# BVE-Reborn/rend3

Hardware: AMD Instinct MI355X
Metric: shaded Mpixels/s @4K (whole frame: cull+compact all cameras, 4 shadow views, PBR opaque, tonemap) (higher is better)
Workload: dtype f32; 1 GPU; BASELINE.json configs[2] stand-in: bistro_like (seed 0xB157, every object owns its geometry), 3840x2160, full PBR opaque + 4 directional shadow views (2048^2), camera dolly, 130 materials with base colour + normal + AO/roughness/metallic maps (RGBA8, mips, trilinear); objects=3000, triangles=2823212, cameras=5, parallelism=single GPU

## Files before the change

### bindings/rend3-amd-sys/src/lib.rs

```rust
#![allow(non_camel_case_types, non_upper_case_globals, clippy::too_many_arguments)]
use std::os::raw::{c_char, c_int, c_void};

pub const R3N_OK: i32 = 0;
pub const R3N_ERR_INVALID_ARG: i32 = -1;
pub const R3N_ERR_HIP: i32 = -2;
pub const R3N_ERR_NO_DEVICE: i32 = -3;
pub const R3N_ERR_STATE: i32 = -4;
pub const R3N_ERR_UNSUPPORTED: i32 = -5;
pub const R3N_ERR_CAPACITY: i32 = -6;
pub const R3N_CAMERA_VIEWPORT: u32 = 0xFFFFFFFF;
pub const R3N_MAX_SHADOW_VIEWS: u32 = 64;
pub const R3N_PASS_DEPTH: u32 = 0;
pub const R3N_PASS_FORWARD: u32 = 1;
pub const R3N_SOURCE_PREDICTED: u32 = 0;
pub const R3N_SOURCE_RESIDUAL: u32 = 1;
pub const R3N_KEY_OPAQUE: u32 = 0;
pub const R3N_KEY_CUTOUT: u32 = 1;
pub const R3N_KEY_BLEND: u32 = 2;
pub const R3N_TEXTURE_RGBA8_UNORM: u32 = 0;
pub const R3N_TEXTURE_RGBA8_UNORM_SRGB: u32 = 1;
pub const R3N_TEXTURE_R8_UNORM: u32 = 2;
pub const R3N_TEXTURE_RG8_UNORM: u32 = 3;
pub const R3N_TEXTURE_BGRA8_UNORM: u32 = 4;
pub const R3N_TEXTURE_BGRA8_UNORM_SRGB: u32 = 5;
// ... 427 lines not shown
    pub fn r3n_output_buffer(ctx: *mut r3n_ctx, rgba8: *mut *mut c_void, bytes: *mut u64) -> c_int;
    pub fn r3n_output_buffer_async(ctx: *mut r3n_ctx, rgba8: *mut *mut c_void, bytes: *mut u64, stream: *mut *mut c_void) -> c_int;
    pub fn r3n_output_work_enqueued(ctx: *mut r3n_ctx) -> c_int;
    pub fn r3n_readback_visible_objects(ctx: *mut r3n_ctx, camera: u32, flags: *mut u8, capacity: u32) -> c_int;
    pub fn r3n_readback_triangle_sets(ctx: *mut r3n_ctx, camera: u32, pass: *mut u8, residual: *mut u8, n: u64) -> c_int;
    pub fn r3n_readback_draw_calls(ctx: *mut r3n_ctx, camera: u32, calls: *mut r3n_indirect_call) -> c_int;
    pub fn r3n_readback_raster_stats(ctx: *mut r3n_ctx, big_items: *mut u32) -> c_int;
    pub fn r3n_readback_blend_order(ctx: *mut r3n_ctx, order: *mut u32, rank_base: *mut u32, capacity: u32) -> c_int;
    pub fn r3n_readback_baked(ctx: *mut r3n_ctx, camera: u32, model_view_and_mvp: *mut f32, capacity: u32) -> c_int;
    pub fn r3n_readback_mesh(ctx: *mut r3n_ctx, byte_offset: u64, dst: *mut c_void, bytes: u64) -> c_int;
    pub fn r3n_readback_joint_matrices(ctx: *mut r3n_ctx, first_matrix: u32, dst: *mut f32, n_matrices: u32) -> c_int;
    pub fn r3n_readback_texture_descs(ctx: *mut r3n_ctx, descs: *mut r3n_texture_desc32, capacity: u32, n_slots: *mut u32) -> c_int;
    pub fn r3n_readback_texels(ctx: *mut r3n_ctx, first_texel: u64, rgba8: *mut u32, n_texels: u64) -> c_int;
    pub fn r3n_readback_visibility(ctx: *mut r3n_ctx, keys: *mut u64) -> c_int;
    pub fn r3n_readback_depth(ctx: *mut r3n_ctx, depth: *mut f32) -> c_int;
    pub fn r3n_readback_hiz(ctx: *mut r3n_ctx, pyramid: *mut f32, count: u64) -> c_int;
    pub fn r3n_readback_shadow_atlas(ctx: *mut r3n_ctx, atlas: *mut f32) -> c_int;
    pub fn r3n_readback_hdr(ctx: *mut r3n_ctx, rgba16f: *mut u16) -> c_int;
    pub fn r3n_readback_output(ctx: *mut r3n_ctx, rgba8: *mut u8, rgba_f32: *mut f32) -> c_int;
    pub fn r3n_timing_enable(ctx: *mut r3n_ctx, enable: c_int) -> c_int;
    pub fn r3n_timing_overhead(ctx: *mut r3n_ctx, ms_per_span: *mut f64) -> c_int;
    pub fn r3n_set_multi_stream(ctx: *mut r3n_ctx, enable: c_int) -> c_int;
    pub fn r3n_stage_times(ctx: *mut r3n_ctx, ms: *mut f64, launches: *mut u64, reset: c_int) -> c_int;
    pub fn r3n_hbm_copy_rate(ctx: *mut r3n_ctx, bytes: u64, repeats: u32, gb_per_s: *mut f64) -> c_int;
    pub fn r3n_selftest_exact_math(hip_device: c_int, hist: *mut u64, guarded: *mut u64) -> c_int;
    pub fn r3n_selftest_unorm8(hip_device: c_int, n_bad: *mut u32) -> c_int;
    pub fn r3n_host_mat4_mul(a: *const f32, b: *const f32, out: *mut f32);
    pub fn r3n_host_mat4_inverse(m: *const f32, out: *mut f32);
    pub fn r3n_host_look_at(eye: *const f32, center: *const f32, up: *const f32, rh: c_int, out: *mut f32);
    pub fn r3n_host_projection(kind: c_int, params: *const f32, rh: c_int, aspect_ratio: f32, out: *mut f32);
    pub fn r3n_host_frustum_from_matrix(m: *const f32, planes20: *mut f32);
    pub fn r3n_host_frustum_contains_sphere(planes20: *const f32, center: *const f32, radius: f32) -> c_int;
    pub fn r3n_host_bounding_sphere_from_mesh(positions: *const f32, vertex_count: u64, out_center: *mut f32, out_radius: *mut f32);
    pub fn r3n_host_bounding_sphere_apply_transform(center: *const f32, radius: f32, m: *const f32, out_center: *mut f32, out_radius: *mut f32);
    pub fn r3n_host_build_object_records(n: u32, transforms: *const f32, mesh_desc: *const f32, mesh_u32: *const u32, material_index: *const u32, out_records: *mut r3n_object128);
    pub fn r3n_host_calculate_normals(positions: *const f32, vertex_count: u64, indices: *const u32, index_count: u64, left_handed: c_int, normals: *mut f32);
    pub fn r3n_host_calculate_tangents(positions: *const f32, normals: *const f32, uvs: *const f32, vertex_count: u64, indices: *const u32, index_count: u64, tangents: *mut f32);
    pub fn r3n_host_vertex_adjacency(indices: *const u32, index_count: u64, vertex_count: u64, out: *mut u32) -> c_int;
    pub fn r3n_host_shadow_camera(direction: *const f32, distance: f32, resolution: u32, camera_location: *const f32, rh: c_int, out_view: *mut f32, out_proj: *mut f32);
    pub fn r3n_host_allocate_shadow_atlas(handles: *const u32, resolutions: *const u16, n: u32, max_dimension: u32, out_dimensions: *mut u32, out_maps: *mut u32) -> u32;
    pub fn r3n_host_evaluate_frame(camera: *const r3n_host_camera144, lights: *const r3n_host_directional_light48, n_lights: u32, max_atlas_dimension: u32, ambient: *const f32, width: u32, height: u32, samples: u32, object_capacity: u32, out: *mut r3n_host_frame) -> c_int;
}
```

### include/r3n.h

```cpp
#ifndef R3N_H
#define R3N_H

#include <stdint.h>

#ifdef __cplusplus
extern "C" {
#endif

#define R3N_OK 0
#define R3N_ERR_INVALID_ARG (-1)
#define R3N_ERR_HIP (-2)
#define R3N_ERR_NO_DEVICE (-3)
#define R3N_ERR_STATE (-4)
#define R3N_ERR_UNSUPPORTED (-5)
#define R3N_ERR_CAPACITY (-6)

typedef uint32_t r3n_camera;
#define R3N_CAMERA_VIEWPORT 0xFFFFFFFFu
#define R3N_MAX_SHADOW_VIEWS 64u

#define R3N_PASS_DEPTH 0u
#define R3N_PASS_FORWARD 1u
#define R3N_SOURCE_PREDICTED 0u
#define R3N_SOURCE_RESIDUAL 1u
// ... 325 lines not shown
#define R3N_STAGE_CLEAR 7
#define R3N_STAGE_RASTER_BIG 8
#define R3N_STAGE_SHADOW_RASTER 9
#define R3N_STAGE_SHADOW_RASTER_BIG 10
#define R3N_STAGE_SKINNING 11
#define R3N_STAGE_VERTEX 12
#define R3N_STAGE_POSE 13
#define R3N_STAGE_EXCHANGE_SHADOW 14
#define R3N_STAGE_EXCHANGE_DEPTH 15
#define R3N_STAGE_EXCHANGE_ROWS 16
#define R3N_STAGE_EXCHANGE_KEYS 17
#define R3N_STAGE_RASTER_CUT 18
#define R3N_STAGE_RASTER_BIG_CUT 19
#define R3N_STAGE_SKYBOX 20
#define R3N_STAGE_BLEND_SORT 21
#define R3N_STAGE_MORPH 22
#define R3N_STAGE_NORMALS 23
#define R3N_STAGE_TANGENTS 24
#define R3N_STAGE_COUNT 25
int r3n_timing_enable(r3n_ctx *ctx, int enable);
int r3n_timing_overhead(r3n_ctx *ctx, double *ms_per_span);
int r3n_set_multi_stream(r3n_ctx *ctx, int enable);
int r3n_stage_times(r3n_ctx *ctx, double ms[R3N_STAGE_COUNT], uint64_t launches[R3N_STAGE_COUNT], int reset);
int r3n_hbm_copy_rate(r3n_ctx *ctx, uint64_t bytes, uint32_t repeats, double *gb_per_s);
int r3n_selftest_exact_math(int hip_device, unsigned long long *hist, unsigned long long *guarded);
int r3n_selftest_unorm8(int hip_device, uint32_t *n_bad);

void r3n_host_mat4_mul(const float *a, const float *b, float *out);
void r3n_host_mat4_inverse(const float *m, float *out);
void r3n_host_look_at(const float eye[3], const float center[3], const float up[3], int rh, float *out);
void r3n_host_projection(int kind, const float *params, int rh, float aspect_ratio, float *out);
void r3n_host_frustum_from_matrix(const float *m, float *planes20);
int r3n_host_frustum_contains_sphere(const float *planes20, const float center[3], float radius);
void r3n_host_bounding_sphere_from_mesh(const float *positions, uint64_t vertex_count, float out_center[3],
                                        float *out_radius);
void r3n_host_bounding_sphere_apply_transform(const float center[3], float radius, const float *m,
                                              float out_center[3], float *out_radius);
void r3n_host_build_object_records(uint32_t n, const float *transforms , const float *mesh_desc ,
                                   const uint32_t *mesh_u32 , const uint32_t *material_index ,
                                   r3n_object128 *out_records);
void r3n_host_calculate_normals(const float *positions, uint64_t vertex_count, const uint32_t *indices,
                                uint64_t index_count, int left_handed, float *normals);
void r3n_host_calculate_tangents(const float *positions, const float *normals, const float *uvs, uint64_t vertex_count,
                                 const uint32_t *indices, uint64_t index_count, float *tangents);
int r3n_host_vertex_adjacency(const uint32_t *indices, uint64_t index_count, uint64_t vertex_count, uint32_t *out);
void r3n_host_shadow_camera(const float direction[3], float distance, uint32_t resolution,
// ... 42 lines not shown
```

### rend3_amd/_ffi.py

```python
import ctypes
import os

import numpy as np

from . import build as _build

vp = ctypes.c_void_p
u32 = ctypes.c_uint32
u64 = ctypes.c_uint64
cint = ctypes.c_int
cfloat = ctypes.c_float

CAMERA_VIEWPORT = 0xFFFFFFFF
PASS_DEPTH, PASS_FORWARD = 0, 1
SOURCE_PREDICTED, SOURCE_RESIDUAL = 0, 1
KEY_OPAQUE, KEY_CUTOUT, KEY_BLEND = 0, 1, 2
STAGES = ["bake", "object_cull", "triangle_cull", "hiz", "raster", "shade", "tonemap", "clear", "raster_big",
          "shadow_raster", "shadow_raster_big", "skinning", "vertex", "pose", "exchange_shadow", "exchange_depth", "exchange_rows", "exchange_keys",
          "raster_cut", "raster_big_cut", "skybox", "blend_sort"]
STAGE_NAMES = STAGES + ["morph", "normals"]
STAGE_TABLE = STAGE_NAMES + ["tangents"]

COMM_ID_BYTES, COMM_IDS = 128, 3

# ... 53 lines not shown
    "r3n_exchange_depth": (cint, [vp, vp, vp]),
    "r3n_set_row_range": (cint, [vp, u32, u32]),
    "r3n_output_buffer": (cint, [vp, vp, vp]),
    "r3n_output_buffer_async": (cint, [vp, vp, vp, vp]),
    "r3n_output_work_enqueued": (cint, [vp]),
    "r3n_readback_visible_objects": (cint, [vp, u32, vp, u32]),
    "r3n_readback_triangle_sets": (cint, [vp, u32, vp, vp, u64]),
    "r3n_readback_draw_calls": (cint, [vp, u32, vp]),
    "r3n_readback_raster_stats": (cint, [vp, vp]),
    "r3n_readback_blend_order": (cint, [vp, vp, vp, u32]),
    "r3n_readback_baked": (cint, [vp, u32, vp, u32]),
    "r3n_readback_mesh": (cint, [vp, u64, vp, u64]),
    "r3n_readback_texture_descs": (cint, [vp, vp, u32, vp]),
    "r3n_readback_texels": (cint, [vp, u64, vp, u64]),
    "r3n_readback_joint_matrices": (cint, [vp, u32, vp, u32]),
    "r3n_readback_visibility": (cint, [vp, vp]),
    "r3n_readback_depth": (cint, [vp, vp]),
    "r3n_readback_hiz": (cint, [vp, vp, u64]),
    "r3n_readback_shadow_atlas": (cint, [vp, vp]),
    "r3n_readback_hdr": (cint, [vp, vp]),
    "r3n_readback_output": (cint, [vp, vp, vp]),
    "r3n_timing_enable": (cint, [vp, cint]),
    "r3n_stage_times": (cint, [vp, vp, vp, cint]),
    "r3n_set_multi_stream": (cint, [vp, cint]),
    "r3n_hbm_copy_rate": (cint, [vp, u64, u32, vp]),
    "r3n_selftest_exact_math": (cint, [cint, vp, vp]),
    "r3n_selftest_unorm8": (cint, [cint, vp]),
    "r3n_host_mat4_mul": (None, [vp, vp, vp]),
    "r3n_host_mat4_inverse": (None, [vp, vp]),
    "r3n_host_look_at": (None, [vp, vp, vp, cint, vp]),
    "r3n_host_projection": (None, [cint, vp, cint, cfloat, vp]),
    "r3n_host_frustum_from_matrix": (None, [vp, vp]),
    "r3n_host_frustum_contains_sphere": (cint, [vp, vp, cfloat]),
    "r3n_host_bounding_sphere_from_mesh": (None, [vp, u64, vp, vp]),
    "r3n_host_bounding_sphere_apply_transform": (None, [vp, cfloat, vp, vp, vp]),
    "r3n_host_build_object_records": (None, [u32, vp, vp, vp, vp, vp]),
    "r3n_host_calculate_normals": (None, [vp, u64, vp, u64, cint, vp]),
    "r3n_host_calculate_tangents": (None, [vp, vp, vp, u64, vp, u64, vp]),
    "r3n_host_vertex_adjacency": (cint, [vp, u64, u64, vp]),
    "r3n_host_shadow_camera": (None, [vp, cfloat, u32, vp, cint, vp, vp]),
    "r3n_host_allocate_shadow_atlas": (u32, [vp, vp, u32, u32, vp, vp]),
    "r3n_host_evaluate_frame": (cint, [vp, vp, u32, u32, vp, u32, u32, u32, u32, vp]),
}

MAX_SHADOW_VIEWS = 64
MAX_MORPH_TARGETS = 256
# ... 90 lines not shown
```

### rend3_amd/csrc/kernels_shade.h

```cpp
#pragma once
#include <type_traits>

#include "device_math.h"
#include "texture.h"

#define R3N_TEX_OCC 5
#define R3N_MS_OCC 4

struct TriRecord;
struct ViewLights;
struct ShadeArgs {
    const unsigned long long *vis;
    uint32_t width, height, row_begin, row_end;
    const r3n_frame_uniforms496 *fu;
    const r3n_camera_header240 *hdr;
    const r3n_object128 *objects;
    const uint32_t *mesh;
    const r3n_baked128 *baked;
    const r3n_material208 *materials;
    uint32_t n_materials;
    const uint32_t *tri_base;
    const uint32_t *slot_table;
    uint32_t slot_table_size;
    const uint8_t *dir_buf;
    const uint8_t *point_buf;
    const float *atlas;
    uint32_t atlas_w, atlas_h;
    float clear[4];
    ushort4 *hdr_out;
    uchar4 *ldr_out;
    const unsigned char *srgb_lut;
    bool out_bgr;
    TextureArgs tex;
    ushort4 *samples_out;
    TriRecord *tri_rec;
    unsigned char *seen;
    uint32_t total_tris;
    uint32_t *edge_list, *edge_count;
    uint32_t edge_capacity;
    const ViewLights *view_lights;
    const uint32_t *material_feat;
    uint32_t variants;
    uint32_t resolve_lds;
};
#define R3N_EDGEQ 32u

#define R3N_FEAT_TEX_ALBEDO   0x001u
#define R3N_FEAT_TEX_NORMAL   0x002u
#define R3N_FEAT_TEX_AOMR     0x004u
#define R3N_FEAT_TEX_AOMR_X   0x008u
#define R3N_FEAT_TEX_MISC     0x010u
#define R3N_FEAT_VCOLOR       0x020u
#define R3N_FEAT_UNLIT        0x040u
#define R3N_FEAT_NEAREST      0x080u
#define R3N_FEAT_AOMR_SPLIT   0x100u
#define R3N_FEAT_CLEARCOAT    0x200u
#define R3N_FEAT_NORMAL_FLAGS 0x400u
#define R3N_FEAT_ALBEDO_OFF   0x800u
#define R3N_FEAT_TEX_GENERAL  0x1000u
#define R3N_FEAT_ALL          0x1FFFu
#define R3N_BATCH_OCC 4
#define R3N_CLS_PLAIN  0u
#define R3N_CLS_ALBEDO (R3N_FEAT_TEX_ALBEDO)
#define R3N_CLS_PBR3   (R3N_FEAT_TEX_ALBEDO | R3N_FEAT_TEX_NORMAL | R3N_FEAT_TEX_AOMR)
#define R3N_CLS_ALL    R3N_FEAT_ALL
#define R3N_VARIANTS 4u
static inline uint32_t r3n_material_features(const r3n_material208 &m) {
    const uint32_t f = m.flags;
// ... 228 lines not shown
R3N_DEV uchar4 tonemap_half4(const unsigned char *__restrict__ lut, ushort4 h, bool bgr = false) {
    const float al = (float)__builtin_bit_cast(_Float16, h.w);
    const float a = (!(al > 0.0f)) ? 0.0f : (al >= 1.0f ? 1.0f : al);
    const unsigned char r = srgb8_of_half(lut, h.x), g = srgb8_of_half(lut, h.y), b = srgb8_of_half(lut, h.z);
    return make_uchar4(bgr ? b : r, g, bgr ? r : b, (unsigned char)(a * 255.0f + 0.5f));
}
R3N_DEV float srgb_scene_to_display(float x) {
    const float e = x > 0.0031308f ? 1.055f * powf(x, 0.4166f) - 0.055f : x * 12.92f;
    if (!(e > 0.0f)) return 0.0f;
    return e >= 1.0f ? 1.0f : e;
}

R3N_DEV ushort4 pack_half4(const float v[4]) {
    ushort4 o;
    o.x = __builtin_bit_cast(unsigned short, (_Float16)v[0]);
    o.y = __builtin_bit_cast(unsigned short, (_Float16)v[1]);
    o.z = __builtin_bit_cast(unsigned short, (_Float16)v[2]);
    o.w = __builtin_bit_cast(unsigned short, (_Float16)v[3]);
    return o;
}


template <bool TEX>
R3N_DEV void vertex_stage(const ShadeArgs &a, uint32_t id, TriRecord &r) {
    const uint32_t slot = id - 1u;
    const uint32_t bucket = slot >> R3N_SLOT_TABLE_SHIFT;
    uint32_t lo = a.slot_table[bucket];
    uint32_t hi = bucket + 1u < a.slot_table_size ? a.slot_table[bucket + 1u] + 1u : a.hdr->object_count;
    while (hi - lo > 1u) {
        const uint32_t mid = lo + (hi - lo) / 2u;
        if (a.tri_base[mid] <= slot) lo = mid; else hi = mid;
    }
    const uint32_t obj = lo, tri = slot - a.tri_base[obj];
    const r3n_object128 &ob = a.objects[obj];
    const uint4 of0 = *reinterpret_cast<const uint4 *>(reinterpret_cast<const char *>(&ob) + 80);
    const uint4 of1 = *reinterpret_cast<const uint4 *>(reinterpret_cast<const char *>(&ob) + 96);
    const uint32_t of5 = ob.vertex_attribute_start_offsets[5];
    const uint32_t mat_index = of0.z < a.n_materials ? of0.z : 0u;
    const r3n_material208 &mat = a.materials[mat_index];
    const float *mv = a.baked[obj].model_view;
    r.object = obj;
    r.material = mat_index;
    r.feat = a.material_feat != nullptr ? a.material_feat[mat_index] : R3N_FEAT_ALL;

    uint32_t idx[3];
    float p[3][4];
    const float inv_s2[3] = {1.0f / dot3(mv, mv), 1.0f / dot3(mv + 4, mv + 4), 1.0f / dot3(mv + 8, mv + 8)};
    const uint32_t first = of0.x + tri * 3u;
    const uint32_t pos_off = of0.w;
    const uint32_t nrm_off = of1.x;
    const uint32_t tan_off = of1.y;
    const uint32_t uv0_off = of1.z;
    const uint32_t col_off = of5;
    bool any_tex = false, normal_map = false;
    if (TEX) {
        const uint4 t0 = *reinterpret_cast<const uint4 *>(&mat.textures[0]), t1 = *reinterpret_cast<const uint4 *>(&mat.textures[4]);
// ... 22 lines not shown
        } else {
            r.vt[k][0] = r.vt[k][1] = r.vt[k][2] = 0.0f;
        }
        if (col_off != R3N_INVALID) {
            const uint32_t cw = a.mesh[col_off / 4u + idx[k]];
#pragma unroll
            for (int c = 0; c < 4; ++c) r.vc[k][c] = (float)((cw >> (8 * c)) & 0xFFu) / 255.0f;
        } else {
#pragma unroll
            for (int c = 0; c < 4; ++c) r.vc[k][c] = 1.0f;
        }
        if (TEX && any_tex) fetch_uv0(a.mesh, uv0_off, idx[k], r.uv[k]);
        else r.uv[k][0] = r.uv[k][1] = 0.0f;
    }
    TriSetup ts;
    setup_triangle(p, (float)a.width / 2.0f, (float)a.height / 2.0f,
                   (a.hdr->flags & R3N_PCU_POSITIVE_AREA_VISIBLE) != 0u, ts);
#pragma unroll
    for (int i = 0; i < 3; ++i)
#pragma unroll
        for (int c = 0; c < 3; ++c) r.e[i][c] = ts.e[i][c];
}

template <class M> R3N_DEV f2 interp2(const float lam[3], f2 a0, f2 a1, f2 a2) {
    return M::mad(splat2(lam[2]), a2, M::mad(splat2(lam[1]), a1, splat2(lam[0]) * a0));
}
template <class M> R3N_DEV float interp1(const float lam[3], float a0, float a1, float a2) {
    return M::mad(lam[2], a2, M::mad(lam[1], a1, lam[0] * a0));
}
template <class M> R3N_DEV void interp_vec3(const float lam[3], const float a[3][3], float o[3]) {
    const f2 xy = interp2<M>(lam, (f2){a[0][0], a[0][1]}, (f2){a[1][0], a[1][1]}, (f2){a[2][0], a[2][1]});
    o[0] = xy.x; o[1] = xy.y;
    o[2] = interp1<M>(lam, a[0][2], a[1][2], a[2][2]);
}
template <class M> R3N_DEV void interp_vec4(const float lam[3], const float a[3][4], float o[4]) {
    const f2 xy = interp2<M>(lam, (f2){a[0][0], a[0][1]}, (f2){a[1][0], a[1][1]}, (f2){a[2][0], a[2][1]});
    const f2 zw = interp2<M>(lam, (f2){a[0][2], a[0][3]}, (f2){a[1][2], a[1][3]}, (f2){a[2][2], a[2][3]});
    o[0] = xy.x; o[1] = xy.y; o[2] = zw.x; o[3] = zw.y;
}

template <class T, bool SL> R3N_DEV T load_light(const T *p) {
#if defined(__HIP_DEVICE_COMPILE__)
    if (SL) {
        static_assert(sizeof(T) % 4 == 0, "whole dwords");
        const unsigned long long v = (unsigned long long)p;
        const uint32_t lo = (uint32_t)__builtin_amdgcn_readfirstlane((uint32_t)v), hi = (uint32_t)__builtin_amdgcn_readfirstlane((uint32_t)(v >> 32));
// ... 258 lines not shown
R3N_DEV void shade_fragment(const ShadeArgs &a, const LdsDirLight *s_dir, const LdsPointLight *s_point, uint32_t n_dir,
                            uint32_t n_point, uint32_t id, uint32_t x, uint32_t y, float out[4]) {
    TriRecord r;
    vertex_stage<TEX>(a, id, r);
    fragment_stage<TEX, M>(a, s_dir, s_point, n_dir, n_point, r, x, y, out);
}

static __global__ __launch_bounds__(256) void k_mark_visible(const unsigned long long *__restrict__ vis, unsigned char *__restrict__ seen,
                                                      size_t first_pixel, size_t n_pixels) {
    const size_t i = (size_t)blockIdx.x * 256u + threadIdx.x;
    const uint32_t id = i < n_pixels ? (uint32_t)(vis[first_pixel + i] & 0xFFFFFFFFull) : 0u;
    const uint32_t left = (uint32_t)__builtin_amdgcn_update_dpp((int)~id, (int)id, 0x111, 0xF, 0xF, false);
    if (id != 0u && id != left) seen[id - 1u] = 1;
}
template <bool TEX>
__global__ __launch_bounds__(256) void k_vertex_stage(ShadeArgs a) {
    const uint32_t slot = blockIdx.x * 256u + threadIdx.x;
    if (slot >= a.total_tris || !a.seen[slot]) return;
    a.seen[slot] = 0;
    TriRecord r;
    vertex_stage<TEX>(a, slot + 1u, r);
    r._pad[0] = r._pad[1] = r._pad[2] = r._pad[3] = 0u;
    a.tri_rec[slot] = r;
}

R3N_DEV void stage_lights(const ShadeArgs &a, LdsDirLight *s_dir, LdsPointLight *s_point, uint32_t &n_dir, uint32_t &n_point) {
    n_dir = min(*reinterpret_cast<const uint32_t *>(a.dir_buf), (uint32_t)R3N_MAX_DIR_LIGHTS);
    n_point = min(*reinterpret_cast<const uint32_t *>(a.point_buf), (uint32_t)R3N_MAX_POINT_LIGHTS);

    const r3n_dir_light128 *dirs = reinterpret_cast<const r3n_dir_light128 *>(a.dir_buf + 16);
    const r3n_point_light32 *points = reinterpret_cast<const r3n_point_light32 *>(a.point_buf + 16);
    for (uint32_t i = threadIdx.x; i < n_dir * 4u; i += 256u) {
        const uint32_t li = i >> 2, c = i & 3u;
        const float *col = a.fu->inv_view + 4 * c;
        float o[4];
        mul_vec4(dirs[li].view_proj, col[0], col[1], col[2], col[3], o);
#pragma unroll
        for (int r = 0; r < 4; ++r) s_dir[li].m[4 * c + r] = o[r];
        if (c == 0) {
            const float nd[3] = {-dirs[li].direction[0], -dirs[li].direction[1], -dirs[li].direction[2]};
            float l[3];
            mat3_mul_vec3(a.fu->view, a.fu->view + 4, a.fu->view + 8, nd, l);
            normalize3(l);
#pragma unroll
            for (int r = 0; r < 3; ++r) { s_dir[li].l[r] = l[r]; s_dir[li].color[r] = dirs[li].color[r]; }
            s_dir[li].sane = (fabsf(dirs[li].color[0]) <= 1e6f && fabsf(dirs[li].color[1]) <= 1e6f && fabsf(dirs[li].color[2]) <= 1e6f &&
// ... 349 lines not shown
    } else {
        h[0] = hdr[i0];
        h[1] = two ? hdr[i0 + 1u] : make_ushort4(0, 0, 0, 0);
    }
    uchar4 o8[2];
#pragma unroll
    for (int k = 0; k < 2; ++k) {
        o8[k] = tonemap_half4(srgb_lut, h[k], bgr);
        if (out_f32 != nullptr && (k == 0 || two)) {
            const float r = (float)__builtin_bit_cast(_Float16, h[k].x), g = (float)__builtin_bit_cast(_Float16, h[k].y);
            const float b = (float)__builtin_bit_cast(_Float16, h[k].z), al = (float)__builtin_bit_cast(_Float16, h[k].w);
            out_f32[i0 + (size_t)k] = make_float4(manual ? srgb_scene_to_display(r) : srgb_oetf(r), manual ? srgb_scene_to_display(g) : srgb_oetf(g),
                                                  manual ? srgb_scene_to_display(b) : srgb_oetf(b),
                                                  (!(al > 0.0f)) ? 0.0f : (al >= 1.0f ? 1.0f : al));
        }
    }
    out[i0] = o8[0];
    if (two) out[i0 + 1u] = o8[1];
}
#endif

extern "C" {
int r3n_internal_build_srgb_lut(unsigned char *lut, hipStream_t stream);
int r3n_internal_shade_prepass(const ShadeArgs *a, int tex, size_t first_key, size_t n_keys, hipStream_t stream);
int r3n_internal_resolve(const ShadeArgs *a, uint32_t samples, int tex, int rec, int split, int fast, hipStream_t stream);
int r3n_internal_resolve_class(const ShadeArgs *a, uint32_t variant, int fast, hipStream_t stream);
int r3n_internal_blend_apply(const ShadeArgs *a, const BlendApplyArgs *b, uint32_t samples, int tex, hipStream_t stream);
int r3n_internal_resolve_samples(const ushort4 *samples, ushort4 *hdr_out, size_t first_pixel, size_t n_pixels, hipStream_t stream);
int r3n_internal_tonemap(const ushort4 *hdr, uchar4 *out, float4 *out_f32, size_t first_pixel, size_t n_pixels, const unsigned char *srgb_lut,
                         uint32_t output_format, hipStream_t stream);
}
```

### rend3_amd/csrc/r3n.hip

```cpp
#include <fcntl.h>
#include <hip/hip_runtime.h>
#include <time.h>
#include <unistd.h>

#include <algorithm>
#include <atomic>
#include <cstdio>
#include <cstdlib>
#include <cstring>
#include <map>
#include <string>
#include <vector>

#include "comm.h"
#include "kernels_cull.h"
#include "kernels_raster.h"
#define R3N_SHADE_DECL_ONLY
#include "kernels_shade.h"
#include "skybox.h"
#include "blend_sort.h"
#include "morph.h"
#include "normals.h"
#include "tangents.h"
#include "texel_alloc.h"
// ... 44 lines not shown
#define R3N_SMALL_GRID 2048
#define R3N_BIG_LDS 40960
#define R3N_SMALL_LDS 24576
#define R3N_VIEWPORT_BIG_LDS 49152
#define R3N_QLANES R3N_AUX_STREAMS
static_assert(R3N_AUX_STREAMS >= 1, "the shadow views draw on auxiliary streams");

struct r3n_ctx {
    int device = 0;
    hipStream_t stream = nullptr;
    hipStream_t aux[R3N_AUX_STREAMS] = {};
    hipEvent_t fork_ev[R3N_AUX_STREAMS] = {};
    hipStream_t shade = nullptr;
    hipEvent_t vp_ev = nullptr, shade_done[2] = {nullptr, nullptr};
    bool shade_pending[2] = {false, false};
    bool shade_unjoined = false;
    int shade_last = 0;
    int slot = 0;
    uint64_t frame_no = 0;
    bool overlap = true;
    bool always_fork = false;
    bool resolve_classes = true;
    bool fused_frame = false;
    DevBuf alt_vis, alt_atlas, alt_vp_baked;
    static constexpr size_t kFbUniforms = 0, kFbViewportHdr = 512, kFbDir = 768, kFbShadowHdr = 3072,
                            kFbPoint = kFbShadowHdr + 256 * R3N_MAX_SHADOW_VIEWS, kFbBytes = kFbPoint + 8448;
    static constexpr int kFbHost = 4;
    DevBuf fb_dev[2];
    uint8_t *fb_host[kFbHost] = {};
    hipEvent_t fb_ev[kFbHost] = {};
    bool fb_pending[kFbHost] = {};
    uint64_t main_epoch = 1, lane_epoch[R3N_AUX_STREAMS] = {};
    DevBuf big_count_all;
    std::vector<uint8_t> h_dir, h_point;
    uint64_t lights_version = 1, slot_lights_version[2] = {0, 0};
    hipEvent_t join_ev[R3N_AUX_STREAMS] = {};
    bool aux_used[R3N_AUX_STREAMS] = {};
    bool multi_stream = true;
    std::string err;
    DevBuf mesh, objects, materials, material_keys, dir_buf, point_buf, fu;
    DevBuf spheres, obj_meta;
    bool meta_dirty = false;
    uint32_t capacity = 0, n_materials = 0;
    std::vector<uint32_t> h_ntri;
    std::vector<uint32_t> h_material;
    std::vector<uint8_t> h_material_key;
// ... 622 lines not shown
        hipEventCreateWithFlags(&c->stage_half_done[1], hipEventDisableTiming) != hipSuccess) {
        g_create_error = "pinned staging ring allocation failed";
        r3n_destroy(c);
        return nullptr;
    }
    if (hipHostMalloc((void **)&c->status_host, 64, hipHostMallocMapped) != hipSuccess ||
        hipHostGetDevicePointer((void **)&c->status_dev, c->status_host, 0) != hipSuccess) {
        g_create_error = "host-mapped status word allocation failed";
        r3n_destroy(c);
        return nullptr;
    }
    c->status_host[0] = 0u;
    if (const char *eb = std::getenv("R3N_BREADCRUMBS")) {
        static std::atomic<int> n_ctx{0};
        const std::string path = std::string(eb) + ".pid" + std::to_string((long long)getpid()) + ".ctx" + std::to_string(n_ctx.fetch_add(1));
        c->crumb_fd = open(path.c_str(), O_CREAT | O_WRONLY | O_APPEND, 0644);
        crumb(c, "created");
    }
    if (const char *es = std::getenv("R3N_SYNC_STAGES")) c->sync_stages = es[0] == '1';
    if (const char *e1 = std::getenv("R3N_SINGLE_STREAM")) c->multi_stream = !(e1[0] == '1');
    if (const char *e2 = std::getenv("R3N_PIPELINE")) c->overlap = !(e2[0] == '0');
    if (const char *e5 = std::getenv("R3N_RESOLVE_CLASSES")) c->resolve_classes = !(e5[0] == '0');
    if (const char *e6 = std::getenv("R3N_ALWAYS_FORK")) c->always_fork = e6[0] == '1';
    if (const char *e3 = std::getenv("R3N_EDGE_CAPACITY")) c->edge_capacity_override = (uint32_t)std::strtoul(e3, nullptr, 10);
    if (const char *e7 = std::getenv("R3N_BIG_CAPACITY"))
        if (const uint32_t n = (uint32_t)std::strtoul(e7, nullptr, 10)) c->big_capacity = n;
    if (const char *e8 = std::getenv("R3N_FRAG_CAPACITY"))
        if (const uint32_t n = (uint32_t)std::strtoul(e8, nullptr, 10)) c->frag_capacity = n;
    if (hipStreamCreateWithPriority(&c->shade, hipStreamNonBlocking, (int)c->tune.prio_shade - 1) != hipSuccess ||
        hipEventCreateWithFlags(&c->vp_ev, hipEventDisableTiming) != hipSuccess ||
        hipEventCreateWithFlags(&c->shade_done[0], hipEventDisableTiming) != hipSuccess ||
        hipEventCreateWithFlags(&c->shade_done[1], hipEventDisableTiming) != hipSuccess) {
        g_create_error = "shade stream creation failed";
        r3n_destroy(c);
        return nullptr;
    }
    for (int k = 0; k < R3N_AUX_STREAMS; ++k)
        if (hipStreamCreateWithPriority(&c->aux[k], hipStreamNonBlocking, (int)c->tune.prio_aux - 1) != hipSuccess ||
            hipEventCreateWithFlags(&c->fork_ev[k], hipEventDisableTiming) != hipSuccess ||
            hipEventCreateWithFlags(&c->join_ev[k], hipEventDisableTiming) != hipSuccess) {
            g_create_error = "auxiliary stream creation failed";
            r3n_destroy(c);
            return nullptr;
        }
    {
        hipStream_t order[2 + R3N_AUX_STREAMS] = {c->stream, c->shade};
// ... 1406 lines not shown
    a.slot_table = c->slot_table.as<uint32_t>();
    a.slot_table_size = c->slot_table_size;
    a.dir_buf = c->dir_buf.as<uint8_t>();
    a.point_buf = c->point_buf.as<uint8_t>();
    a.atlas = c->atlas.as<float>();
    a.atlas_w = std::max(1u, c->atlas_w); a.atlas_h = std::max(1u, c->atlas_h);
    std::memcpy(a.clear, c->clear, 16);
    a.hdr_out = c->hdr16.as<ushort4>();
    a.ldr_out = c->out8.as<uchar4>();
    a.srgb_lut = c->srgb_lut.as<unsigned char>();
    a.out_bgr = (c->output_format & 1u) != 0u;
    a.tex = texture_args(c);
    a.samples_out = nullptr;
    a.tri_rec = nullptr;
    a.seen = nullptr;
    a.resolve_lds = c->tune.resolve_lds;
    a.total_tris = (uint32_t)c->total_tris;
    a.view_lights = nullptr;
    a.material_feat = nullptr;
    a.variants = 0u;
    return a;
}

int r3n_resolve_opaque(r3n_ctx *c) {
    if (!c || !c->in_frame) return fail(c, R3N_ERR_STATE, "resolve_opaque: outside a frame");
    HIP_TRY(c, hipSetDevice(c->device));
    const uint32_t r0 = std::min(c->row_begin, c->height), r1 = std::min(c->row_end, c->height);
    c->sky_window = r1 <= r0;
    c->resolve_on_shade = false;
    if (r1 <= r0) return R3N_OK;
    CamState &s = c->viewport;
    if (!s.has_hdr && c->capacity) return fail(c, R3N_ERR_STATE, "resolve_opaque: viewport uniforms not baked");
    const bool use_records = c->total_tris > 0 && (uint64_t)c->total_tris * sizeof(TriRecord) <= (8ull << 30);
    const uint64_t npix_all = (uint64_t)c->width * c->height;
    const bool blend_samples = c->samples == 4 && c->blend_tris > 0;
    const bool split = c->samples == 4 && use_records && !blend_samples && npix_all < (1ull << 29);
    uint32_t edge_cap = 0;
    const bool classes = use_records && c->samples == 1 && c->n_textures > 0 && c->n_materials > 0 && c->resolve_classes;
    if (classes) TRY(refresh_material_classes(c));
    if (use_records && c->samples == 1) TRY(ensure(c, c->view_lights[c->slot], sizeof(ViewLights), false, -1));
    if (use_records) {
        TRY(ensure(c, c->tri_rec, (size_t)c->total_tris * sizeof(TriRecord), false, -1));
        TRY(ensure(c, c->tri_seen, (size_t)c->total_tris, false, 0));
    }
    const bool sky = c->sky_cube != 0u;
    const bool sky_samples = sky && c->samples == 4 && !split && !blend_samples;
    if (blend_samples || split || sky_samples) TRY(ensure(c, c->samples16, (size_t)npix_all * 4 * 8, false, -1));
    if (split) {
        edge_cap = (uint32_t)((uint64_t)(r1 - r0) * c->width * 3u / R3N_EDGEQ) + 4096u;
        if (c->edge_capacity_override) edge_cap = c->edge_capacity_override;
        TRY(ensure(c, c->edge_list, (size_t)edge_cap * R3N_EDGEQ * 4, false, -1));
        TRY(ensure(c, c->edge_count, R3N_EDGEQ * 4, false, 0));
    }
    const bool on_shade = c->overlap && c->multi_stream && (!c->timing || c->tune.timed_pipeline != 0u) && c->blend_tris == 0;
    hipStream_t stream = on_shade ? c->shade : c->stream;
    if (on_shade) {
        HIP_TRY(c, hipEventRecord(c->vp_ev, c->stream));
        HIP_TRY(c, hipStreamWaitEvent(c->shade, c->vp_ev, 0));
        for (int k = 0; k < R3N_AUX_STREAMS; ++k)
            if (c->aux_used[k]) {
                HIP_TRY(c, hipEventRecord(c->join_ev[k], c->aux[k]));
                HIP_TRY(c, hipStreamWaitEvent(c->shade, c->join_ev[k], 0));
            }
    } else {
        TRY(join_lanes(c));
        TRY(join_shade(c));
    }
    ShadeArgs a = make_shade_args(c, r0, r1);
    if (blend_samples || sky_samples) a.samples_out = c->samples16.as<ushort4>();
    if (use_records && c->samples == 1) a.view_lights = c->view_lights[c->slot].as<ViewLights>();
    if (classes && c->resolve_variants != 0u) {
        a.material_feat = c->material_feat.as<uint32_t>();
        a.variants = c->resolve_variants;
    }
    c->resolved_this_frame = true;
    const bool tex = c->n_textures > 0;
    if (use_records) {
        a.tri_rec = c->tri_rec.as<TriRecord>();
        a.seen = c->tri_seen.as<unsigned char>();
        Timed t(c, R3N_STAGE_VERTEX, stream);
        const size_t first = (size_t)r0 * c->width * c->samples, npx = (size_t)(r1 - r0) * c->width * c->samples;
        HIP_TRY(c, (hipError_t)r3n_internal_shade_prepass(&a, tex ? 1 : 0, first, npx, stream));
    }
    {
        Timed t(c, R3N_STAGE_SHADE, stream);
        if (split) {
            a.samples_out = c->samples16.as<ushort4>();
            a.edge_list = c->edge_list.as<uint32_t>();
            a.edge_count = c->edge_count.as<uint32_t>();
            a.edge_capacity = edge_cap;
            HIP_TRY(c, hipMemsetAsync(a.edge_count, 0, R3N_EDGEQ * 4, stream));
        }
        HIP_TRY(c, (hipError_t)r3n_internal_resolve(&a, c->samples, tex ? 1 : 0, a.tri_rec != nullptr ? 1 : 0, split ? (sky ? 2 : 1) : 0,
                                                    c->shade_mode == R3N_SHADE_FAST ? 1 : 0, stream));
    }
    TRY(check_launch(c, "k_resolve_opaque"));
    if (on_shade) {
        HIP_TRY(c, hipEventRecord(c->shade_done[c->slot], c->shade));
        c->shade_pending[c->slot] = true;
        c->shade_unjoined = true;
        c->shade_last = c->slot;
    }
    c->sky_window = true;
    c->resolve_on_shade = on_shade;
    c->sky_samples_form = split ? R3N_SKY_SAMPLES_EDGES : R3N_SKY_SAMPLES_ALL;
// ... 569 lines not shown
        return fail(c, R3N_ERR_INVALID_ARG, "render_frame: null uniforms / headers, or too many shadow views");
    if (c->in_frame) return fail(c, R3N_ERR_STATE, "render_frame: a frame is already open");
    const bool native = c->comm.on;
    crumb(c, "render_frame", d->width, d->height);
    if (native) {
        if (d->exchange) return fail(c, R3N_ERR_INVALID_ARG, "render_frame: an exchange callback AND r3n_comm_init communicators");
        band_rows(d->height, c->comm.world, c->comm.rank, c->row_begin, c->row_end);
    }
    for (uint32_t v = 0; v < d->n_shadow_views; ++v)
        if (d->shadow_views[v].header.shadow_index != v) return fail(c, R3N_ERR_INVALID_ARG, "render_frame: shadow view i must carry shadow_index i");
    if (d->directional_buffer) TRY(r3n_lights_write(c, d->directional_buffer, d->directional_bytes, d->point_buffer, d->point_bytes));
    TRY(frame_begin_impl(c, d->uniforms, d->width, d->height, d->samples, d->clear_color, d->shadow_atlas_width, d->shadow_atlas_height, d));
    c->viewport.hdr_frame = c->frame_no;
    for (uint32_t v = 0; v < d->n_shadow_views; ++v)
        if (CamState *s = find_cam(c, v, true)) {
            s->hdr_frame = c->frame_no;
            s->d_hdr.p = c->fb_dev[c->slot].as<uint8_t>() + r3n_ctx::kFbShadowHdr + 256u * (size_t)v;
            s->d_hdr.bytes = 256;
        }
    struct Closer {
        r3n_ctx *c; bool armed = true;
        ~Closer() { if (armed && c->in_frame) { const std::string keep = c->err; (void)close_frame(c); c->err = keep; } }
    } closer{c};
    struct Fused { r3n_ctx *c; ~Fused() { c->fused_frame = false; } } fused{c};
    c->fused_frame = true;
    const bool masked = native || (d->flags & R3N_FRAME_SHADOW_MASK) != 0u;
    auto mine = [&](uint32_t v) {
        if (native) return shadow_part_of(c->comm.world, d->n_shadow_views, c->comm.rank, v) >= 0;
        return !masked || ((d->shadow_view_mask >> v) & 1ull) != 0ull;
    };
    for (uint32_t v = 0; v < d->n_shadow_views; ++v) {
        const r3n_shadow_view272 &sv = d->shadow_views[v];
        TRY(r3n_shadow_viewport(c, v, sv.x, sv.y, sv.size));
        {
            CamState *s = find_cam(c, v, true);
            if (!s) return fail(c, R3N_ERR_INVALID_ARG, "render_frame: bad shadow camera");
            s->band_begin = 0; s->band_end = 0xFFFFFFFFu;
            const int part = native ? shadow_part_of(c->comm.world, d->n_shadow_views, c->comm.rank, v) : -1;
            if (part >= 0) band_rows(sv.size, shadow_parts(c->comm.world, d->n_shadow_views), (uint32_t)part, s->band_begin, s->band_end);
        }
        if (masked) TRY(r3n_set_camera_object_range(c, v, mine(v) ? 0u : 0xFFFFFFFFu, mine(v) ? 0xFFFFFFFEu : 0xFFFFFFFFu));
    }
    if (d->n_skeletons) TRY(r3n_skinning(c, d->skin_inputs, d->n_skeletons, d->joint_matrices, d->n_joint_matrices));
    auto shadow_nodes = [&]() -> int {
        for (uint32_t v = 0; v < d->n_shadow_views; ++v)
            if (mine(v)) TRY(r3n_uniform_bake(c, v, &d->shadow_views[v].header));
        for (uint32_t v = 0; v < d->n_shadow_views; ++v)
            if (mine(v)) TRY(r3n_cull(c, v));
// ... 456 lines not shown
                c->hbm_best_variant = v;
            }
        }
    }
    if (e0) (void)hipEventDestroy(e0);
    if (e1) (void)hipEventDestroy(e1);
    if (a) (void)hipFree(a);
    if (b) (void)hipFree(b);
    if (rc == R3N_OK) *gb_per_s = best > 0.0f ? 2.0 * (double)(n * 16) / ((double)best * 1e-3) / 1e9 : 0.0;
    if (rc == R3N_OK && std::getenv("R3N_VERBOSE")) std::fprintf(stderr, "r3n_hbm_copy_rate: best variant %d (kernel %d, grid %u): %.1f GB/s\n", c->hbm_best_variant, c->hbm_best_variant / 4, c->hbm_best_variant < 24 ? 256u * (4u << (c->hbm_best_variant % 4)) : 0u, *gb_per_s);
    return rc;
}

int r3n_stage_times(r3n_ctx *c, double ms[R3N_STAGE_COUNT], uint64_t launches[R3N_STAGE_COUNT], int reset) {
    if (!c) return R3N_ERR_INVALID_ARG;
    TRY(drain_timing(c));
    for (int i = 0; i < R3N_STAGE_COUNT; ++i) {
        if (ms) ms[i] = c->stage_ms[i];
        if (launches) launches[i] = c->stage_launches[i];
        if (reset) { c->stage_ms[i] = 0; c->stage_launches[i] = 0; }
    }
    return R3N_OK;
}

}
```

### rend3_amd/csrc/shade.hip

```cpp
#include <hip/hip_runtime.h>

#include "kernels_shade.h"

namespace {
int launch_status() { return (int)hipGetLastError(); }
}

extern "C" int r3n_internal_resolve_ms(const ShadeArgs *ap, int tex, int rec, int split, hipStream_t stream);

extern "C" {

int r3n_internal_build_srgb_lut(unsigned char *lut, hipStream_t stream) {
    hipLaunchKernelGGL(k_build_srgb_lut, dim3((R3N_SRGB_LUT_SIZE + 255u) / 256u), dim3(256), 0, stream, lut);
    return launch_status();
}

int r3n_internal_shade_prepass(const ShadeArgs *ap, int tex, size_t first_key, size_t n_keys, hipStream_t stream) {
    const ShadeArgs &a = *ap;
    hipLaunchKernelGGL(k_mark_visible, dim3((unsigned)((n_keys + 255) / 256)), dim3(256), 0, stream, a.vis, a.seen, first_key, n_keys);
    const dim3 vgrid((unsigned)(((size_t)a.total_tris + 255) / 256));
    if (tex) hipLaunchKernelGGL(k_vertex_stage<true>, vgrid, dim3(256), 0, stream, a);
    else hipLaunchKernelGGL(k_vertex_stage<false>, vgrid, dim3(256), 0, stream, a);
    return launch_status();
}

int r3n_internal_resolve(const ShadeArgs *ap, uint32_t samples, int tex, int rec, int split, int fast, hipStream_t stream) {
    if (samples == 4) return r3n_internal_resolve_ms(ap, tex, rec, split, stream);
    const ShadeArgs &a = *ap;
    const dim3 rgrid((a.width + 15u) / 16u, (a.row_end - a.row_begin + 15u) / 16u);
    if (rec) {
        if (!a.view_lights) return (int)hipErrorInvalidValue;
        hipLaunchKernelGGL(k_stage_view_lights, dim3(1), dim3(256), 0, stream, a, const_cast<ViewLights *>(a.view_lights));
    }
    if (rec && tex && a.variants != 0u) {
        for (uint32_t v = 0; v < R3N_VARIANTS; ++v) {
            if (!((a.variants >> v) & 1u)) continue;
            if (v < R3N_VARIANTS - 1u) {
                const int rc = r3n_internal_resolve_class(ap, v, fast, stream);
                if (rc) return rc;
            } else if (fast) {
                hipLaunchKernelGGL((k_resolve_opaque<1, true, true, false, true>), rgrid, dim3(256), a.resolve_lds, stream, a);
// ... 27 lines not shown
```

### rend3_amd/renderer.py

```python
import ctypes

import os

import numpy as np

from . import _ffi, host

f32 = np.float32
INVALID = 0xFFFFFFFF
OPAQUE, CUTOUT, BLEND = 0, 1, 2

FLAGS_ALBEDO_ACTIVE = 0x0001
FLAGS_ALBEDO_BLEND = 0x0002
FLAGS_ALBEDO_VERTEX_SRGB = 0x0004
FLAGS_AOMR_COMBINED = 0x0040
FLAGS_AOMR_SPLIT = 0x0100
FLAGS_CC_GLTF_COMBINED = 0x0400
FLAGS_BICOMPONENT_NORMAL = 0x0008
FLAGS_SWIZZLED_NORMAL = 0x0010
FLAGS_YDOWN_NORMAL = 0x0020
FLAGS_AOMR_SWIZZLED_SPLIT = 0x0080
FLAGS_AOMR_BW_SPLIT = 0x0200
FLAGS_CC_GLTF_SPLIT = 0x0800
FLAGS_CC_BW_SPLIT = 0x1000
# ... 1126 lines not shown
        n = 0
        k = 0
        m = max(width, height)
        while m:
            n += max(1, width >> k) * max(1, height >> k)
            k += 1
            m >>= 1
        pyr = np.zeros(n, dtype=f32)
        self._check(self.lib.r3n_readback_hiz(self.ctx, _ffi.ptr(pyr), n), "readback_hiz")
        return pyr

    def timing_enable(self, on=True):
        self._check(self.lib.r3n_timing_enable(self.ctx, 1 if on else 0), "r3n_timing_enable")

    def set_multi_stream(self, on=True):
        self._check(self.lib.r3n_set_multi_stream(self.ctx, 1 if on else 0), "r3n_set_multi_stream")

    def stage_times(self, reset=True):
        ms = np.zeros(len(_ffi.STAGE_TABLE), dtype=np.float64)
        n = np.zeros(len(_ffi.STAGE_TABLE), dtype=np.uint64)
        self._check(self.lib.r3n_stage_times(self.ctx, _ffi.ptr(ms), _ffi.ptr(n), 1 if reset else 0), "r3n_stage_times")
        return {s: (float(ms[i]), int(n[i])) for i, s in enumerate(_ffi.STAGE_TABLE)}

    def hbm_copy_rate(self, nbytes=1 << 30, repeats=5):
        out = ctypes.c_double(0.0)
        self._check(self.lib.r3n_hbm_copy_rate(self.ctx, int(nbytes), int(repeats), ctypes.byref(out)), "r3n_hbm_copy_rate")
        return float(out.value)

    def sync(self):
        self._check(self.lib.r3n_sync(self.ctx), "r3n_sync")


class RenderGraph:

    def __init__(self):
        self.nodes = []

    def add_node(self, name, body):
        self.nodes.append((name, body))

    def execute(self, renderer, eval_output):
        for _name, body in self.nodes:
            body(renderer, eval_output)


class BaseRenderGraphSettings:
# ... 171 lines not shown
```

Before: 9454 Mpixels/s.

## Build triangle shading records from culled draw lists instead of scanning all triangles

Measured after the change: 9544 Mpixels/s, median of 6. About the same (+1.0%).

```diff
diff --git a/bindings/rend3-amd-sys/src/lib.rs b/bindings/rend3-amd-sys/src/lib.rs
--- a/bindings/rend3-amd-sys/src/lib.rs
+++ b/bindings/rend3-amd-sys/src/lib.rs
@@ -473,6 +473,7 @@
     pub fn r3n_timing_overhead(ctx: *mut r3n_ctx, ms_per_span: *mut f64) -> c_int;
     pub fn r3n_set_multi_stream(ctx: *mut r3n_ctx, enable: c_int) -> c_int;
     pub fn r3n_stage_times(ctx: *mut r3n_ctx, ms: *mut f64, launches: *mut u64, reset: c_int) -> c_int;
+    pub fn r3n_record_frames(ctx: *mut r3n_ctx, from_lists: *mut u64, from_flags: *mut u64, reset: c_int) -> c_int;
     pub fn r3n_hbm_copy_rate(ctx: *mut r3n_ctx, bytes: u64, repeats: u32, gb_per_s: *mut f64) -> c_int;
     pub fn r3n_selftest_exact_math(hip_device: c_int, hist: *mut u64, guarded: *mut u64) -> c_int;
     pub fn r3n_selftest_unorm8(hip_device: c_int, n_bad: *mut u32) -> c_int;
diff --git a/include/r3n.h b/include/r3n.h
--- a/include/r3n.h
+++ b/include/r3n.h
@@ -371,6 +371,7 @@
 int r3n_timing_overhead(r3n_ctx *ctx, double *ms_per_span);
 int r3n_set_multi_stream(r3n_ctx *ctx, int enable);
 int r3n_stage_times(r3n_ctx *ctx, double ms[R3N_STAGE_COUNT], uint64_t launches[R3N_STAGE_COUNT], int reset);
+int r3n_record_frames(r3n_ctx *ctx, uint64_t *from_lists, uint64_t *from_flags, int reset);
 int r3n_hbm_copy_rate(r3n_ctx *ctx, uint64_t bytes, uint32_t repeats, double *gb_per_s);
 int r3n_selftest_exact_math(int hip_device, unsigned long long *hist, unsigned long long *guarded);
 int r3n_selftest_unorm8(int hip_device, uint32_t *n_bad);
diff --git a/rend3_amd/_ffi.py b/rend3_amd/_ffi.py
--- a/rend3_amd/_ffi.py
+++ b/rend3_amd/_ffi.py
@@ -99,6 +99,7 @@
     "r3n_readback_output": (cint, [vp, vp, vp]),
     "r3n_timing_enable": (cint, [vp, cint]),
     "r3n_stage_times": (cint, [vp, vp, vp, cint]),
+    "r3n_record_frames": (cint, [vp, vp, vp, cint]),
     "r3n_set_multi_stream": (cint, [vp, cint]),
     "r3n_hbm_copy_rate": (cint, [vp, u64, u32, vp]),
     "r3n_selftest_exact_math": (cint, [cint, vp, vp]),
diff --git a/rend3_amd/csrc/kernels_shade.h b/rend3_amd/csrc/kernels_shade.h
--- a/rend3_amd/csrc/kernels_shade.h
+++ b/rend3_amd/csrc/kernels_shade.h
@@ -44,6 +44,12 @@
     uint32_t resolve_lds;
 };
 #define R3N_EDGEQ 32u
+struct RecordLists {
+    const r3n_tri_ref *list[2];
+    const uint32_t *sub_counts[2];
+    uint32_t subcap[2];
+};
+#define R3N_RECORD_LIST_BLOCKS 32u
 
 #define R3N_FEAT_TEX_ALBEDO   0x001u
 #define R3N_FEAT_TEX_NORMAL   0x002u
@@ -318,16 +324,7 @@
 
 
 template <bool TEX>
-R3N_DEV void vertex_stage(const ShadeArgs &a, uint32_t id, TriRecord &r) {
-    const uint32_t slot = id - 1u;
-    const uint32_t bucket = slot >> R3N_SLOT_TABLE_SHIFT;
-    uint32_t lo = a.slot_table[bucket];
-    uint32_t hi = bucket + 1u < a.slot_table_size ? a.slot_table[bucket + 1u] + 1u : a.hdr->object_count;
-    while (hi - lo > 1u) {
-        const uint32_t mid = lo + (hi - lo) / 2u;
-        if (a.tri_base[mid] <= slot) lo = mid; else hi = mid;
-    }
-    const uint32_t obj = lo, tri = slot - a.tri_base[obj];
+R3N_DEV void vertex_stage_of(const ShadeArgs &a, uint32_t obj, uint32_t tri, TriRecord &r) {
     const r3n_object128 &ob = a.objects[obj];
     const uint4 of0 = *reinterpret_cast<const uint4 *>(reinterpret_cast<const char *>(&ob) + 80);
     const uint4 of1 = *reinterpret_cast<const uint4 *>(reinterpret_cast<const char *>(&ob) + 96);
@@ -396,6 +393,23 @@
         for (int c = 0; c < 3; ++c) r.e[i][c] = ts.e[i][c];
 }
 
+R3N_DEV uint32_t slot_object(const ShadeArgs &a, uint32_t slot) {
+    const uint32_t bucket = slot >> R3N_SLOT_TABLE_SHIFT;
+    uint32_t lo = a.slot_table[bucket];
+    uint32_t hi = bucket + 1u < a.slot_table_size ? a.slot_table[bucket + 1u] + 1u : a.hdr->object_count;
+    while (hi - lo > 1u) {
+        const uint32_t mid = lo + (hi - lo) / 2u;
+        if (a.tri_base[mid] <= slot) lo = mid; else hi = mid;
+    }
+    return lo;
+}
+template <bool TEX>
+R3N_DEV void vertex_stage(const ShadeArgs &a, uint32_t id, TriRecord &r) {
+    const uint32_t slot = id - 1u;
+    const uint32_t obj = slot_object(a, slot);
+    vertex_stage_of<TEX>(a, obj, slot - a.tri_base[obj], r);
+}
+
 template <class M> R3N_DEV f2 interp2(const float lam[3], f2 a0, f2 a1, f2 a2) {
     return M::mad(splat2(lam[2]), a2, M::mad(splat2(lam[1]), a1, splat2(lam[0]) * a0));
 }
@@ -700,6 +714,35 @@
     vertex_stage<TEX>(a, slot + 1u, r);
     r._pad[0] = r._pad[1] = r._pad[2] = r._pad[3] = 0u;
     a.tri_rec[slot] = r;
+}
+template <bool TEX>
+__global__ __launch_bounds__(256) void k_vertex_stage_lists(ShadeArgs a, RecordLists l) {
+    const uint32_t q = blockIdx.x % R3N_SUBQ;
+    const uint32_t n0 = l.list[0] ? min(l.sub_counts[0][R3N_KEY_OPAQUE * R3N_SUBQ + q], l.subcap[0]) : 0u;
+    const uint32_t n1 = l.list[0] ? min(l.sub_counts[0][R3N_KEY_CUTOUT * R3N_SUBQ + q], l.subcap[0]) : 0u;
+    const uint32_t n2 = l.list[1] ? min(l.sub_counts[1][R3N_KEY_OPAQUE * R3N_SUBQ + q], l.subcap[1]) : 0u;
+    const uint32_t n3 = l.list[1] ? min(l.sub_counts[1][R3N_KEY_CUTOUT * R3N_SUBQ + q], l.subcap[1]) : 0u;
+    const uint32_t e0 = n0, e1 = e0 + n1, e2 = e1 + n2, e3 = e2 + n3;
+    const uint32_t object_count = a.hdr->object_count;
+    const uint32_t stride = (gridDim.x / R3N_SUBQ) * 256u;
+    for (uint32_t i = (blockIdx.x / R3N_SUBQ) * 256u + threadIdx.x; i < e3; i += stride) {
+        const uint32_t src = i < e1 ? 0u : 1u, key = (i < e0 || (i >= e1 && i < e2)) ? R3N_KEY_OPAQUE : R3N_KEY_CUTOUT;
+        const uint32_t j = i - (i < e0 ? 0u : i < e1 ? e0 : i < e2 ? e1 : e2);
+        const r3n_tri_ref ref = l.list[src][(size_t)(key * R3N_SUBQ + q) * l.subcap[src] + j];
+        const uint32_t obj = ref.object;
+        if (a.objects[obj].enabled == 0u) continue;
+        const uint32_t slot = a.tri_base[obj] + ref.triangle;
+        if (slot >= a.total_tris) continue;
+        uint32_t o = obj, tri = ref.triangle;
+        if (!(obj < object_count && (obj + 1u == object_count || slot < a.tri_base[obj + 1u]))) {
+            o = slot_object(a, slot);
+            tri = slot - a.tri_base[o];
+        }
+        TriRecord r;
+        vertex_stage_of<TEX>(a, o, tri, r);
+        r._pad[0] = r._pad[1] = r._pad[2] = r._pad[3] = 0u;
+        a.tri_rec[slot] = r;
+    }
 }
 
 R3N_DEV void stage_lights(const ShadeArgs &a, LdsDirLight *s_dir, LdsPointLight *s_point, uint32_t &n_dir, uint32_t &n_point) {
@@ -1095,7 +1138,7 @@
 
 extern "C" {
 int r3n_internal_build_srgb_lut(unsigned char *lut, hipStream_t stream);
-int r3n_internal_shade_prepass(const ShadeArgs *a, int tex, size_t first_key, size_t n_keys, hipStream_t stream);
+int r3n_internal_shade_prepass(const ShadeArgs *a, const RecordLists *lists, int tex, size_t first_key, size_t n_keys, hipStream_t stream);
 int r3n_internal_resolve(const ShadeArgs *a, uint32_t samples, int tex, int rec, int split, int fast, hipStream_t stream);
 int r3n_internal_resolve_class(const ShadeArgs *a, uint32_t variant, int fast, hipStream_t stream);
 int r3n_internal_blend_apply(const ShadeArgs *a, const BlendApplyArgs *b, uint32_t samples, int tex, hipStream_t stream);
diff --git a/rend3_amd/csrc/r3n.hip b/rend3_amd/csrc/r3n.hip
--- a/rend3_amd/csrc/r3n.hip
+++ b/rend3_amd/csrc/r3n.hip
@@ -90,6 +90,9 @@
     bool always_fork = false;
     bool resolve_classes = true;
     bool fused_frame = false;
+    bool frame_exchange = false;
+    bool records_from_lists = true;
+    uint64_t record_frames[2] = {0, 0};
     DevBuf alt_vis, alt_atlas, alt_vp_baked;
     static constexpr size_t kFbUniforms = 0, kFbViewportHdr = 512, kFbDir = 768, kFbShadowHdr = 3072,
                             kFbPoint = kFbShadowHdr + 256 * R3N_MAX_SHADOW_VIEWS, kFbBytes = kFbPoint + 8448;
@@ -758,6 +761,7 @@
     if (const char *e2 = std::getenv("R3N_PIPELINE")) c->overlap = !(e2[0] == '0');
     if (const char *e5 = std::getenv("R3N_RESOLVE_CLASSES")) c->resolve_classes = !(e5[0] == '0');
     if (const char *e6 = std::getenv("R3N_ALWAYS_FORK")) c->always_fork = e6[0] == '1';
+    if (const char *e8 = std::getenv("R3N_RECORDS_FROM_LISTS")) c->records_from_lists = !(e8[0] == '0');
     if (const char *e3 = std::getenv("R3N_EDGE_CAPACITY")) c->edge_capacity_override = (uint32_t)std::strtoul(e3, nullptr, 10);
     if (const char *e7 = std::getenv("R3N_BIG_CAPACITY"))
         if (const uint32_t n = (uint32_t)std::strtoul(e7, nullptr, 10)) c->big_capacity = n;
@@ -2210,6 +2214,22 @@
     return a;
 }
 
+static RecordLists record_lists(const CamState &s) {
+    RecordLists l{};
+    if (s.has_prev) {
+        const int idx = 1 - s.cur;
+        l.list[0] = s.predicted[idx].as<r3n_tri_ref>();
+        l.sub_counts[0] = &s.sub_counts[idx].as<r3n_sub_counts>()->n[0][0][0];
+        l.subcap[0] = s.subcap[idx];
+    }
+    if (s.culled) {
+        l.list[1] = s.residual.as<r3n_tri_ref>();
+        l.sub_counts[1] = &s.sub_counts[s.cur].as<r3n_sub_counts>()->n[1][0][0];
+        l.subcap[1] = s.subcap[s.cur];
+    }
+    return l;
+}
+
 int r3n_resolve_opaque(r3n_ctx *c) {
     if (!c || !c->in_frame) return fail(c, R3N_ERR_STATE, "resolve_opaque: outside a frame");
     HIP_TRY(c, hipSetDevice(c->device));
@@ -2227,6 +2247,7 @@
     const bool classes = use_records && c->samples == 1 && c->n_textures > 0 && c->n_materials > 0 && c->resolve_classes;
     if (classes) TRY(refresh_material_classes(c));
     if (use_records && c->samples == 1) TRY(ensure(c, c->view_lights[c->slot], sizeof(ViewLights), false, -1));
+    const bool from_lists = use_records && c->records_from_lists && c->fused_frame && !c->frame_exchange && !c->comm.on && c->blend_tris == 0;
     if (use_records) {
         TRY(ensure(c, c->tri_rec, (size_t)c->total_tris * sizeof(TriRecord), false, -1));
         TRY(ensure(c, c->tri_seen, (size_t)c->total_tris, false, 0));
@@ -2268,7 +2289,9 @@
         a.seen = c->tri_seen.as<unsigned char>();
         Timed t(c, R3N_STAGE_VERTEX, stream);
         const size_t first = (size_t)r0 * c->width * c->samples, npx = (size_t)(r1 - r0) * c->width * c->samples;
-        HIP_TRY(c, (hipError_t)r3n_internal_shade_prepass(&a, tex ? 1 : 0, first, npx, stream));
+        const RecordLists lists = record_lists(s);
+        HIP_TRY(c, (hipError_t)r3n_internal_shade_prepass(&a, from_lists ? &lists : nullptr, tex ? 1 : 0, first, npx, stream));
+        c->record_frames[from_lists ? 0 : 1]++;
     }
     {
         Timed t(c, R3N_STAGE_SHADE, stream);
@@ -2884,8 +2907,9 @@
         r3n_ctx *c; bool armed = true;
         ~Closer() { if (armed && c->in_frame) { const std::string keep = c->err; (void)close_frame(c); c->err = keep; } }
     } closer{c};
-    struct Fused { r3n_ctx *c; ~Fused() { c->fused_frame = false; } } fused{c};
+    struct Fused { r3n_ctx *c; ~Fused() { c->fused_frame = false; c->frame_exchange = false; } } fused{c};
     c->fused_frame = true;
+    c->frame_exchange = d->exchange != nullptr;
     const bool masked = native || (d->flags & R3N_FRAME_SHADOW_MASK) != 0u;
     auto mine = [&](uint32_t v) {
         if (native) return shadow_part_of(c->comm.world, d->n_shadow_views, c->comm.rank, v) >= 0;
@@ -3388,5 +3412,12 @@
     }
     return R3N_OK;
 }
-
-}
+int r3n_record_frames(r3n_ctx *c, uint64_t *from_lists, uint64_t *from_flags, int reset) {
+    if (!c) return R3N_ERR_INVALID_ARG;
+    if (from_lists) *from_lists = c->record_frames[0];
+    if (from_flags) *from_flags = c->record_frames[1];
+    if (reset) c->record_frames[0] = c->record_frames[1] = 0;
+    return R3N_OK;
+}
+
+}
diff --git a/rend3_amd/csrc/shade.hip b/rend3_amd/csrc/shade.hip
--- a/rend3_amd/csrc/shade.hip
+++ b/rend3_amd/csrc/shade.hip
@@ -15,8 +15,14 @@
     return launch_status();
 }
 
-int r3n_internal_shade_prepass(const ShadeArgs *ap, int tex, size_t first_key, size_t n_keys, hipStream_t stream) {
+int r3n_internal_shade_prepass(const ShadeArgs *ap, const RecordLists *lists, int tex, size_t first_key, size_t n_keys, hipStream_t stream) {
     const ShadeArgs &a = *ap;
+    if (lists) {
+        const dim3 lgrid(R3N_SUBQ * R3N_RECORD_LIST_BLOCKS);
+        if (tex) hipLaunchKernelGGL(k_vertex_stage_lists<true>, lgrid, dim3(256), 0, stream, a, *lists);
+        else hipLaunchKernelGGL(k_vertex_stage_lists<false>, lgrid, dim3(256), 0, stream, a, *lists);
+        return launch_status();
+    }
     hipLaunchKernelGGL(k_mark_visible, dim3((unsigned)((n_keys + 255) / 256)), dim3(256), 0, stream, a.vis, a.seen, first_key, n_keys);
     const dim3 vgrid((unsigned)(((size_t)a.total_tris + 255) / 256));
     if (tex) hipLaunchKernelGGL(k_vertex_stage<true>, vgrid, dim3(256), 0, stream, a);
diff --git a/rend3_amd/renderer.py b/rend3_amd/renderer.py
--- a/rend3_amd/renderer.py
+++ b/rend3_amd/renderer.py
@@ -1172,6 +1172,11 @@
         self._check(self.lib.r3n_stage_times(self.ctx, _ffi.ptr(ms), _ffi.ptr(n), 1 if reset else 0), "r3n_stage_times")
         return {s: (float(ms[i]), int(n[i])) for i, s in enumerate(_ffi.STAGE_TABLE)}
 
+    def record_frames(self, reset=False):
+        a, b = ctypes.c_uint64(0), ctypes.c_uint64(0)
+        self._check(self.lib.r3n_record_frames(self.ctx, ctypes.byref(a), ctypes.byref(b), 1 if reset else 0), "r3n_record_frames")
+        return int(a.value), int(b.value)
+
     def hbm_copy_rate(self, nbytes=1 << 30, repeats=5):
         out = ctypes.c_double(0.0)
         self._check(self.lib.r3n_hbm_copy_rate(self.ctx, int(nbytes), int(repeats), ctypes.byref(out)), "r3n_hbm_copy_rate")
```
